# albertgassol1/vf-nerf

Hardware: AMD Instinct MI355X
Metric: rays/sec (4096-ray chunk, 128 samples/ray) + PSNR vs ref (higher is better)
Workload: dtype f16x3+f32acc

## Files before the change

### vf_nerf_amd/csrc/vfn_mlp16.hip

```cpp
#include <string.h>
#include <utility>
#include "vfn_common.h"
#include "vfn_plan.h"

typedef _Float16 half8 __attribute__((ext_vector_type(8)));
typedef _Float16 half2v __attribute__((ext_vector_type(2)));
typedef float float2v __attribute__((ext_vector_type(2)));
typedef float f32x16 __attribute__((ext_vector_type(16)));
typedef float f32x4v __attribute__((ext_vector_type(4)));

#ifndef VFN16_ASCALE
#define VFN16_ASCALE 1
#endif
#define VFN16_WSCALE 64.0f
#define VFN16_INV_WSCALE 0.015625f
#define VFN16_PACK_WSCALE (VFN16_ASCALE ? 1.0f : VFN16_WSCALE)
#define VFN16_XSCALE (VFN16_ASCALE ? VFN16_WSCALE : 1.0f)
#ifndef VFN16_SAVE_AUX
#define VFN16_SAVE_AUX 2
#endif
#ifndef VFN16_HANDOVER_NUM
#define VFN16_HANDOVER_NUM 8
#endif
#ifndef VFN16_DMA_STEPS
#define VFN16_DMA_STEPS 16
#endif
#ifndef VFN16_EPI_PER_MFMA
#define VFN16_EPI_PER_MFMA 6
#endif
#ifndef VFN16_EPI_PER_MFMA2
#define VFN16_EPI_PER_MFMA2 9
#endif
#ifndef VFN16_LATE_STORES
// ... 236 lines not shown
constexpr int rn_off_kb(int h) { int o = 0; for (int i = 0; i < h; ++i) o += RN_TILES[i] * chunk_kb(RN_ACT[i], RN_AUX[i]); return o; }

struct ChunkD { int net, off_kb, kb, aux; };
constexpr ChunkD chunk_of(int mode, int c) {
    if (!(mode & M16_BLKIN)) {
        const int vf_layers = (mode & M16_FEAT) ? 9 : 8;
        for (int h = 0; h < vf_layers; ++h) {
            if (c < VF_TILES[h]) return {0, vf_off_kb(h) + c * chunk_kb(VF_ACT[h], VF_AUX[h]), chunk_kb(VF_ACT[h], VF_AUX[h]), VF_AUX[h]};
            c -= VF_TILES[h];
        }
        if (c == 0) return {0, vf_off_kb(9), HEAD_KB, 0};
        c -= 1;
    }
    if (mode & M16_RENDER) {
        for (int h = 0; h < 4; ++h) {
            if (c < RN_TILES[h]) return {1, rn_off_kb(h) + c * chunk_kb(RN_ACT[h], RN_AUX[h]), chunk_kb(RN_ACT[h], RN_AUX[h]), RN_AUX[h]};
            c -= RN_TILES[h];
        }
        if (c == 0) return {1, rn_off_kb(4), HEAD_KB, 0};
    }
    return {0, 0, 0, 0};
}

constexpr int rn_first_chunk(int mode) { return (mode & M16_BLKIN) ? 0 : 72; }
constexpr bool chunk_two(int mode, int c) { return (mode & M16_C2) && !(mode & M16_BLKIN) && c >= 63 && c != 71; }
constexpr bool mode_one(int mode) { return (mode & M16_P1) != 0; }
#ifndef VFN16_P1_RING
#define VFN16_P1_RING 5
#endif
#define VFN16_P1_SLOT_KB 20
constexpr int ring_of(int mode) { return mode_one(mode) ? VFN16_P1_RING : 3; }
constexpr int slot_u4(int mode) { return mode_one(mode) ? VFN16_P1_SLOT_KB * 64 : VFN16_MAX_CHUNK_KB * 64; }
constexpr int slot_base(int mode, int c) { return (c % ring_of(mode)) * slot_u4(mode); }
static_assert(VFN16_P1_RING * VFN16_P1_SLOT_KB <= 3 * VFN16_MAX_CHUNK_KB, "the single-product ring must fit into the split modes' ring");
constexpr int stores_of(int mode, int c) { return (c == 0 || ((mode & M16_RENDER) && c == rn_first_chunk(mode))) ? 0 : 4; }
constexpr int young_ops(int mode, int c) {
    const int ring = ring_of(mode);
    int n = 0;
    for (int k = (c - ring + 2 > 0 ? c - ring + 2 : 0); k < c; ++k) n += stores_of(mode, k);
    for (int j = 2; j <= ring - 2; ++j)
        if (c + j >= ring - 1 && chunk_of(mode, c + j).kb > 0) n += (((chunk_of(mode, c + j).kb - 1) / 2 + 1) / VFN16_WAVES);
    return n;
}

struct Mlp16Args {
    const uint4* vf_w;
    const uint4* rn_w;
    const float* points;
    const float* ray_dirs;
    float* out_vec;
    float* out_colors;
    long long n_points;
    int dirs_div;
    int vf_multires, rn_multires;
    uint32_t vf_bytes, rn_bytes;
    float* saved;
    float* save_aux_vf;
    float* save_aux_rn;
    uint32_t* save_masks;
    int save_f16;
    uint4* blk_out;
    const uint4* blk_in;
    const float* vec_in;
    const int* src;
    const int* out_index;
    long long ws_first, ws_points;
// ... 164 lines not shown
        typedef unsigned int u32x16 __attribute__((ext_vector_type(16)));
        const u32x16 u = __builtin_bit_cast(u32x16, cy.pend);
        constexpr int N = 16 / PARTS;
        if constexpr (PART == 0) b = 0;
#pragma unroll
        for (int r = 15 - PART * N; r > 15 - (PART + 1) * N; --r) b = __builtin_amdgcn_alignbit(b, u[r] + 0x7fffffffu, 31);
        if constexpr (PART == PARTS - 1) cy.lm[TILE >> 1] |= b << (16 * (TILE & 1));
    }
}
template <int SLOT>
__device__ __forceinline__ void store_mask(const Pipe16& p, Carry16& cy) {
    typedef unsigned int u32x4 __attribute__((ext_vector_type(4)));
    const __amdgpu_buffer_rsrc_t rs = __builtin_amdgcn_make_buffer_rsrc(
        reinterpret_cast<unsigned char*>(p.masks) + (size_t)SLOT * p.mask_bytes, 0, (int)p.mask_bytes, 0x00020000);
    const u32x4 w = {cy.lm[0], cy.lm[1], cy.lm[2], cy.lm[3]};
    __builtin_amdgcn_raw_buffer_store_b128(w, rs, (int)p.mask_voff, 0, 0);
    cy.lm[0] = 0; cy.lm[1] = 0; cy.lm[2] = 0; cy.lm[3] = 0;
}

template <int TILE>
__device__ __forceinline__ void store_blocks(const Pipe16& p, const X16& x) {
    typedef unsigned int u32x4 __attribute__((ext_vector_type(4)));
    const __amdgpu_buffer_rsrc_t rs = __builtin_amdgcn_make_buffer_rsrc(p.blk_out, 0, (int)p.blk_bytes, 0x00020000);
#pragma unroll
    for (int s = 0; s < 2; ++s) {
        __builtin_amdgcn_raw_buffer_store_b128(__builtin_bit_cast(u32x4, x.hi[2 * TILE + s]), rs, (int)p.blk_voff, (2 * TILE + s) * 2048, 0);
        __builtin_amdgcn_raw_buffer_store_b128(__builtin_bit_cast(u32x4, x.lo[2 * TILE + s]), rs, (int)p.blk_voff, (2 * TILE + s) * 2048 + 1024, 0);
    }
}

template <int MODE, int C0, int ACT, int AUX, int NCH, int EPI, int PEPI, int PKB, int SLOT = -1, int PSLOT = -1, bool BLK = false,
          bool PBLK = false>
__device__ __forceinline__ void layer16(const X16& xin, const A16& aux, X16& xout, X16& xpend, Carry16& cy, float (&head)[3],
                                       const Pipe16& p, int wave, int lane) {
    constexpr int NKB = ACT + AUX;
    constexpr int E = NKB / 2 > 0 ? NKB / 2 : 1;
    constexpr int H = NKB * VFN16_HANDOVER_NUM / 16 > 0 ? NKB * VFN16_HANDOVER_NUM / 16 : 1;
    constexpr int PMAX = (VFN16_MAX_CHUNK_KB + VFN16_WAVES - 1) / VFN16_WAVES;
    constexpr int DSPAN = NKB - H > 0 ? NKB - H : 1;
    constexpr int DSTEPS = DSPAN < VFN16_DMA_STEPS ? DSPAN : VFN16_DMA_STEPS;
    static_assert(PEPI < 0 || PKB >= E, "the pending tile must be complete before it is read");
    constexpr bool TRAIN = (MODE & M16_TRAIN) != 0;
    constexpr bool LATE = TRAIN && VFN16_LATE_STORES;
    constexpr int DEND = LATE ? (NKB - 4 > H + 1 ? NKB - 4 : (H + 1 < NKB ? H + 1 : NKB - 1)) : 0;
    constexpr int SBEG = LATE ? DEND : H;
    constexpr int SSTEPS = LATE ? (NKB - DEND > 0 ? NKB - DEND : 1) : (DSPAN < 4 ? DSPAN : 4);
    constexpr int DST = LATE ? (DEND - H > 0 ? DEND - H : 1) : DSTEPS;
    constexpr int MPARTS = (LATE && E <= H) ? (DEND - H >= 4 ? 4 : (DEND - H >= 2 ? 2 : (DEND - H >= 1 ? 1 : 0))) : 0;
    static_for<NCH>([&](auto ich) {
        constexpr int ch = decltype(ich)::value;
        constexpr int C = C0 + ch;
        constexpr int RING = ring_of(MODE);
        constexpr ChunkD dcur = chunk_of(MODE, C), dnext = chunk_of(MODE, C + 1), ddma = chunk_of(MODE, C + RING - 1);
        static_assert(dcur.kb == 2 * NKB + 1, "layer shape and chunk table disagree");
        constexpr bool P1 = mode_one(MODE);
        constexpr bool W2 = chunk_two(MODE, C);
        constexpr bool D2 = chunk_two(MODE, C + RING - 1) || P1;
        constexpr int DNKB = (ddma.kb - 1) / 2;
        constexpr int DPIECES = P1 ? DNKB + 1 : (D2 ? DNKB + ddma.aux + 1 : ddma.kb);
        auto piece_blk = [&](int idx) -> int {
            if (P1) return idx < DNKB ? 2 * idx : 2 * DNKB;
            if (!D2) return idx;
            if (ddma.aux == 0) return 2 * idx;
            return idx < DNKB ? 2 * idx : (idx < DNKB + ddma.aux ? 2 * (idx - ddma.aux) + 1 : 2 * DNKB);
        };
        constexpr int PM = D2 ? (DPIECES + VFN16_WAVES - 1) / VFN16_WAVES : PMAX;
        const uint4* cb = p.lds + slot_base(MODE, C);
        constexpr int FB = P1 ? 1 : 2;
        f32x16 acc = cy.bias;
        half8 fh[VFN16_FDEPTH], fl[VFN16_FDEPTH];
        fh[0] = cy.fh0;
        if (!P1 && (!W2 || ACT == 0)) fl[0] = cy.fl0;
        if (VFN16_FDEPTH == 3 && NKB > 1) {
            fh[1] = __builtin_bit_cast(half8, cb[FB * 64 + lane]);
            if (!W2 && !P1) fl[1] = __builtin_bit_cast(half8, cb[3 * 64 + lane]);
        }
        half8 ehi[2], elo[2];
        [[maybe_unused]] unsigned mbits = 0;
#pragma unroll
        for (int st = 0; st < NKB; ++st) {
            constexpr int AHEAD = VFN16_FDEPTH - 1;
            if (st + AHEAD < NKB) {
                fh[(st + AHEAD) % VFN16_FDEPTH] = __builtin_bit_cast(half8, cb[(FB * (st + AHEAD)) * 64 + lane]);
                if (!P1 && (!W2 || st + AHEAD >= ACT)) fl[(st + AHEAD) % VFN16_FDEPTH] = __builtin_bit_cast(half8, cb[(2 * (st + AHEAD) + 1) * 64 + lane]);
            }
            const half8 a_hi = fh[st % VFN16_FDEPTH];
            const half8 x_hi = st < ACT ? xin.hi[st < ACT ? st : 0] : aux.hi[st >= ACT ? st - ACT : 0];
            const half8 x_lo = st < ACT ? xin.lo[st < ACT ? st : 0] : aux.lo[st >= ACT ? st - ACT : 0];
            acc = __builtin_amdgcn_mfma_f32_32x32x16_f16(a_hi, x_hi, acc, 0, 0, 0);
#ifndef ABL_P1
// ... 4 lines not shown
#endif
#ifdef ABL_NOEPI
            if (st == 0 && (ch > 0 || PEPI >= 0)) asm volatile("" :: "v"(cy.pend));
            if (false) {
#else
            if (st < E && (ch > 0 || PEPI >= 0)) {
#endif
#pragma unroll
                for (int pr = st * 8 / E; pr < (st + 1) * 8 / E; ++pr) {
                    const int sblk = pr >> 2, j = (pr & 3) * 2;
                    if (ch > 0) epi_pair<EPI, TRAIN, !P1>(cy.pend, cy.sat, pr, ehi[sblk], elo[sblk], j);
                    else epi_pair<(PEPI >= 0 ? PEPI : 0), TRAIN, !P1>(cy.pend, cy.sat, pr, ehi[sblk], elo[sblk], j);
                    if ((pr & 3) == 3) {
                        asm volatile("" : "+a"(ehi[sblk]));
                        if constexpr (!P1) asm volatile("" : "+a"(elo[sblk]));
                        if (ch > 0) { xout.hi[2 * (ch > 0 ? ch - 1 : 0) + sblk] = ehi[sblk]; if constexpr (!P1) xout.lo[2 * (ch > 0 ? ch - 1 : 0) + sblk] = elo[sblk]; }
                        else { xpend.hi[PKB + sblk] = ehi[sblk]; if constexpr (!P1) xpend.lo[PKB + sblk] = elo[sblk]; }
                    }
                }
#ifndef VFN16_NOGROUPS
                if constexpr (!P1) {
                __builtin_amdgcn_sched_group_barrier(0x100, W2 ? 1 : 2, 0);
                __builtin_amdgcn_sched_group_barrier(0x008, 1, 0);
                __builtin_amdgcn_sched_group_barrier(0x002, W2 ? VFN16_EPI_PER_MFMA2 : VFN16_EPI_PER_MFMA, 0);
                __builtin_amdgcn_sched_group_barrier(0x008, 1, 0);
                __builtin_amdgcn_sched_group_barrier(0x002, W2 ? VFN16_EPI_PER_MFMA2 : VFN16_EPI_PER_MFMA, 0);
                if (!W2) {
                    __builtin_amdgcn_sched_group_barrier(0x008, 1, 0);
                    __builtin_amdgcn_sched_group_barrier(0x002, VFN16_EPI_PER_MFMA, 0);
                }
                }
#endif
            }
            if (st == H - 1 && dnext.kb > 0) {
#ifndef ABL_NOSYNC
#ifdef ABL_LOOSE_WAIT
                if ((MODE & M16_TRAIN) != 0) asm volatile("s_waitcnt vmcnt(4)" ::: "memory");
                else
#endif
                if constexpr (P1 && LATE) {
                    constexpr int young = young_ops(MODE, C);
                    static_assert(young < 64, "vmcnt is a 6-bit field");
                    if constexpr (young == 0) asm volatile("s_waitcnt vmcnt(0)" ::: "memory");
                    else asm volatile("s_waitcnt vmcnt(%0)" :: "n"(young) : "memory");
                } else
                if (LATE && C > 0 && (ch == 0 || ch > 1 || PEPI >= 0)) asm volatile("s_waitcnt vmcnt(4)" ::: "memory");
                else asm volatile("s_waitcnt vmcnt(0)" ::: "memory");
                __builtin_amdgcn_s_barrier();
#endif
            }
#ifndef ABL_NODMA
            if (st >= H && st < H + DST && ddma.kb > 0) {
#pragma unroll
                for (int i = (st - H) * PM / DST; i < (st - H + 1) * PM / DST; ++i) {
                    if (VFN16_WAVES * i + VFN16_WAVES <= DPIECES) dma_piece<ddma.net, ddma.off_kb, slot_base(MODE, C + RING - 1)>(p, piece_blk(wave + VFN16_WAVES * i), lane, P1 ? wave + VFN16_WAVES * i : -1);
                    else if (VFN16_WAVES * i < DPIECES) {
                        const int idx = min(wave + VFN16_WAVES * i, DPIECES - 1);
                        dma_piece<ddma.net, ddma.off_kb, slot_base(MODE, C + RING - 1)>(p, piece_blk(idx), lane, P1 ? idx : -1);
                    }
                }
            }
#endif
#ifndef ABL_NOMASK
            if (TRAIN && MPARTS > 0 && st >= H && st < H + MPARTS && (ch > 0 || PEPI >= 0)) {
                static_for<MPARTS>([&](auto ip) {
                    constexpr int part = decltype(ip)::value;
                    if (st - H == part) {
                        if (ch > 0) collect_mask_part<(ch > 0 ? ch - 1 : 0), EPI, part, (MPARTS > 0 ? MPARTS : 1)>(cy, mbits);
                        else collect_mask_part<PKB / 2, (PEPI >= 0 ? PEPI : 0), part, (MPARTS > 0 ? MPARTS : 1)>(cy, mbits);
                    }
                });
            }
#endif
            if (TRAIN && st >= SBEG && st < SBEG + SSTEPS && (ch > 0 || PEPI >= 0)) {
#ifndef ABL_NOMASK
                if (st == (LATE ? SBEG : VFN16_MASK_STEP(H, NKB))) {
                    if constexpr (MPARTS > 0) {
                        if (ch == 0) store_mask<(PSLOT >= 0 ? PSLOT : 0)>(p, cy);
                    } else {
                        if (ch > 0) collect_mask<(ch > 0 ? ch - 1 : 0), EPI>(cy);
                        else { collect_mask<PKB / 2, (PEPI >= 0 ? PEPI : 0)>(cy); store_mask<(PSLOT >= 0 ? PSLOT : 0)>(p, cy); }
                    }
                }
#endif
#pragma unroll
                for (int q = (st - SBEG) * 4 / SSTEPS; q < (st - SBEG + 1) * 4 / SSTEPS; ++q) {
                    if (ch > 0) save_group<(SLOT >= 0 ? SLOT : 0), (ch > 0 ? ch - 1 : 0), (MODE & M16_SF16) != 0>(p, cy.pend, q);
                    else save_group<(PSLOT >= 0 ? PSLOT : 0), PKB / 2, (MODE & M16_SF16) != 0>(p, cy.pend, q);
                }
            }
            if (st == H && ((BLK && ch > 0) || (PBLK && ch == 0))) {
                if (ch > 0) store_blocks<(ch > 0 ? ch - 1 : 0)>(p, xout);
                else store_blocks<PKB / 2>(p, xpend);
            }
            if (st == NKB - 1 && dnext.kb > 0) prefetch_chunk<MODE, (dnext.kb > 0 ? C + 1 : C)>(cy, p, lane);
#ifndef VFN16_NOSCHED
            __builtin_amdgcn_sched_barrier(0);
#endif
        }
        if (EPI == EPI_RELU || EPI == EPI_TANH) {
            cy.pend = acc;
#if VFN16_RANGE_TRACK == 2
            if (EPI == EPI_RELU) {
                float mx = fmaxf(acc[0], acc[1]);
#pragma unroll
                for (int r = 2; r < 16; r += 2) mx = fmaxf(mx, fmaxf(acc[r], acc[r + 1]));
                cy.sat |= __builtin_amdgcn_ballot_w64(mx >= VFN16_CLAMP);
            }
#endif
        } else {
#pragma unroll
            for (int c = 0; c < 3; ++c) {
                const float v = acc[c] * VFN16_INV_WSCALE;
                head[c] = (EPI == EPI_HEAD_TANH) ? tanh_exp(v) : 1.0f / (1.0f + expf(-v));
            }
        }
    });
}

__device__ __forceinline__ float enc_value(const float (&x)[3], const float (&sn)[18], const float (&cs)[18], int multires, int k) {
    if (k < 3) return x[k];
    const int idx = k - 3, oct = idx / 6, rem = idx - 6 * oct;
    if (oct >= multires) return 0.f;
    return rem < 3 ? sn[3 * oct + rem] : cs[3 * oct + rem - 3];
}

template <typename F>
__device__ __forceinline__ void build_aux(A16& aux, int g, F col, float& ain) {
// ... 42 lines not shown
#pragma unroll
    for (int j = 0; j < 3; ++j)
#pragma unroll
        for (int c = 0; c < 3; ++c) {
            float s = 0.f, k = 0.f;
            if (2 * j < multires) {
                sincosf(x[c] * (g ? (float)(2 << (2 * j)) : (float)(1 << (2 * j))), &s, &k);
                if (2 * j + g >= multires) { s = 0.f; k = 0.f; }
            }
            const float so = __shfl_xor(s, 32, 64), ko = __shfl_xor(k, 32, 64);
            sn[6 * j + c] = g ? so : s;          cs[6 * j + c] = g ? ko : k;
            sn[6 * j + 3 + c] = g ? s : so;      cs[6 * j + 3 + c] = g ? k : ko;
        }
}

template <int MODE>
__device__ __forceinline__ void render_aux(const Mlp16Args& a, A16& aux, const float (&xr)[3], const float (&dr)[3], const float (&nrm)[3],
                                           long long m, bool in, int g, float& ain) {
    const int rn_multires = a.rn_multires;
    float sn[18], cs[18];
    encode_sincos(dr, rn_multires, g, sn, cs);
    const int ncol = 6 + 6 * rn_multires;
    auto rn_col = [&](int k) -> float {
        if (k < 3) return xr[k];
        if (k >= ncol) return k < ncol + 3 ? nrm[k - ncol] : 0.f;
        return enc_value(dr, sn, cs, rn_multires, k - 3);
    };
    build_aux(aux, g, rn_col, ain);
    if ((MODE & M16_TRAIN) && in) save_aux(a.save_aux_rn, m, g, rn_col);
}

template <int MODE>
__device__ __forceinline__ void render_tail(const Mlp16Args& a, const Pipe16& p, Carry16& cy, X16& xa, X16& xb, const A16& aux,
                                            const float (&nrm)[3], long long m, bool in, int wave, int lane) {
    constexpr int R = EPI_RELU, NONE = -1;
    constexpr int C0 = rn_first_chunk(MODE);
    float rgb[3] = {0.f, 0.f, 0.f};
    layer16<MODE, C0 + 0, 16, 3, 8, R, NONE, 0, 9, -1>(xb, aux, xa, xb, cy, rgb, p, wave, lane);
    layer16<MODE, C0 + 8, 16, 0, 8, R, R, 14, 10, 9>(xa, aux, xb, xa, cy, rgb, p, wave, lane);
    layer16<MODE, C0 + 16, 16, 0, 8, R, R, 14, 11, 10>(xb, aux, xa, xb, cy, rgb, p, wave, lane);
    layer16<MODE, C0 + 24, 16, 0, 8, R, R, 14, 12, 11>(xa, aux, xb, xa, cy, rgb, p, wave, lane);
    layer16<MODE, C0 + 32, 16, 0, 1, EPI_HEAD_SIGMOID, R, 14, -1, 12>(xb, aux, xa, xb, cy, rgb, p, wave, lane);
    const long long mo = m;
    if (in && (threadIdx.x & 32) == 0) {
        a.out_vec[mo * 3 + 0] = nrm[0]; a.out_vec[mo * 3 + 1] = nrm[1]; a.out_vec[mo * 3 + 2] = nrm[2];
        a.out_colors[mo * 3 + 0] = rgb[0]; a.out_colors[mo * 3 + 1] = rgb[1]; a.out_colors[mo * 3 + 2] = rgb[2];
    }
}

__device__ __forceinline__ void report_range(const Mlp16Args& a, unsigned long long sat, float ain) {
    if (a.status) {
        const unsigned bits = (sat != 0ull ? 1u : 0u) | (ain >= VFN16_CLAMP ? 2u : 0u);
        if (bits) atomicOr(a.status, bits);
    }
}

template <int MODE>
__global__ __launch_bounds__(256, 1) void vfn_mlp16_kernel(const Mlp16Args a) {
    __shared__ __attribute__((aligned(16))) uint4 s_ring[3 * VFN16_SLOT + 256 * 8];
    float* s_park = reinterpret_cast<float*>(s_ring + 3 * VFN16_SLOT) + threadIdx.x * 32;
    const int tid = threadIdx.x;
    const int lane = tid & 63;
    const int wave = __builtin_amdgcn_readfirstlane(tid >> 6);
    const int g = lane >> 5;
#ifdef VFN16_STAMPS
    const unsigned long long st_t0 = __builtin_amdgcn_s_memtime(), st_r0 = __builtin_amdgcn_s_memrealtime();
#endif
    unsigned long long ck_t0 = 0ull, ck_r0 = 0ull;
    if constexpr ((MODE & M16_RENDER) != 0 && (MODE & M16_BLKIN) == 0 && (MODE & M16_TRAIN) == 0) {
        if (a.clock) { ck_t0 = __builtin_amdgcn_s_memtime(); ck_r0 = __builtin_amdgcn_s_memrealtime(); }
    }
    const long long m = (long long)blockIdx.x * VFN16_PTS + wave * 32 + (lane & 31);
    long long n_live = a.n_points;
    if (a.n_dev) {
        const long long nd = (long long)*a.n_dev;
        n_live = nd < n_live ? nd : n_live;
        if ((long long)blockIdx.x * VFN16_PTS >= n_live) return;
    }
    const bool in = m < n_live;

    if constexpr ((MODE & M16_BLKIN) != 0) {
        const int dpos = in ? a.src[m] : -1;
        const bool live = dpos >= 0;
        float xr[3] = {0.f, 0.f, 0.f}, dr[3] = {0.f, 0.f, 0.f}, nrm[3] = {0.f, 0.f, 0.f};
        if (live) {
            const long long di = dpos / a.dirs_div;
#pragma unroll
            for (int c = 0; c < 3; ++c) { xr[c] = a.points[(long long)dpos * 3 + c]; dr[c] = a.ray_dirs[di * 3 + c]; nrm[c] = a.vec_in[m * 3 + c]; }
        }
        Pipe16 p;
        p.lds = s_ring;
        p.vf_w = __builtin_amdgcn_make_buffer_rsrc(const_cast<uint4*>(a.rn_w), 0, (int)a.rn_bytes, 0x00020000);
        p.rn_w = p.vf_w;
        p.saved = nullptr; p.slot_floats = 0; p.slot_bytes = 0; p.save_voff = 0; p.blk_out = nullptr; p.blk_bytes = 0; p.blk_voff = 0;
        p.masks = nullptr; p.mask_bytes = 0; p.mask_voff = 0; p.save16 = 0; p.save_voff16 = 0; p.feat_voff = 0; p.st_tile = 0; p.st_q = 0;
        dma_chunk<MODE, 0>(p, wave, lane);
        dma_chunk<MODE, 1>(p, wave, lane);
        X16 xa, xb;
        A16 aux;
        float ain_blk = 0.f;
        {
            typedef unsigned int u32x4 __attribute__((ext_vector_type(4)));
            const __amdgpu_buffer_rsrc_t rs_blk = __builtin_amdgcn_make_buffer_rsrc(
                const_cast<uint4*>(a.blk_in), 0, (int)(((a.n_points + 31) & ~31ll) * 1024), 0x00020000);
            const unsigned goff = in ? (unsigned)((m >> 5) * 32768 + lane * 16) : 0xfffffff0u;
            u32x4 q[32];
#pragma unroll
            for (int i = 0; i < 32; ++i) q[i] = __builtin_amdgcn_raw_buffer_load_b128(rs_blk, goff, i * 1024, 0);
            render_aux<MODE>(a, aux, xr, dr, nrm, -1, false, g, ain_blk);
#pragma unroll
            for (int t = 0; t < 8; ++t) {
                half8 h0 = __builtin_bit_cast(half8, q[4 * t + 0]), l0 = __builtin_bit_cast(half8, q[4 * t + 1]);
                half8 h1 = __builtin_bit_cast(half8, q[4 * t + 2]), l1 = __builtin_bit_cast(half8, q[4 * t + 3]);
                asm volatile("" : "+a"(h0)); asm volatile("" : "+a"(l0)); asm volatile("" : "+a"(h1)); asm volatile("" : "+a"(l1));
                xb.hi[2 * t] = h0; xb.lo[2 * t] = l0; xb.hi[2 * t + 1] = h1; xb.lo[2 * t + 1] = l1;
            }
        }
        asm volatile("s_waitcnt vmcnt(0)" ::: "memory");
        __builtin_amdgcn_s_barrier();
        Carry16 cy;
#pragma unroll
        for (int q = 0; q < 16; ++q) cy.pend[q] = 0.f;
        cy.lm[0] = 0; cy.lm[1] = 0; cy.lm[2] = 0; cy.lm[3] = 0; cy.sat = 0ull;
        prefetch_chunk<MODE, 0>(cy, p, lane);
#ifdef VFN16_STAMPS
        const unsigned long long st_t1 = __builtin_amdgcn_s_memtime();
#endif
        render_tail<MODE>(a, p, cy, xa, xb, aux, nrm, live ? (long long)dpos : -1, live, wave, lane);
        report_range(a, cy.sat, ain_blk);
#ifdef VFN16_STAMPS
        if (threadIdx.x == 0 && live) {
            const unsigned long long t2 = __builtin_amdgcn_s_memtime(), r2 = __builtin_amdgcn_s_memrealtime();
            a.out_colors[(long long)dpos * 3 + 0] = (float)(st_t1 - st_t0); a.out_colors[(long long)dpos * 3 + 1] = (float)(t2 - st_t0);
            a.out_colors[(long long)dpos * 3 + 2] = (float)(r2 - st_r0);
        }
#endif
    } else {
    float x[3] = {0.f, 0.f, 0.f};
    if (in) { x[0] = a.points[m * 3 + 0]; x[1] = a.points[m * 3 + 1]; x[2] = a.points[m * 3 + 2]; }
    float d[3] = {0.f, 0.f, 0.f};
    int out_row = -1;
    if ((MODE & M16_RENDER) && in) {
        const long long di = m / a.dirs_div;
        d[0] = a.ray_dirs[di * 3 + 0]; d[1] = a.ray_dirs[di * 3 + 1]; d[2] = a.ray_dirs[di * 3 + 2];
        if (a.out_index) out_row = a.out_index[m];
    }
    asm volatile("s_waitcnt vmcnt(0)" ::: "memory");
    if (MODE & M16_RENDER) {
        s_park[0] = x[0]; s_park[1] = x[1]; s_park[2] = x[2];
        s_park[4] = d[0]; s_park[5] = d[1]; s_park[6] = d[2];
    }

    Pipe16 p;
    p.lds = s_ring;
    p.vf_w = __builtin_amdgcn_make_buffer_rsrc(const_cast<uint4*>(a.vf_w), 0, (int)a.vf_bytes, 0x00020000);
    p.rn_w = __builtin_amdgcn_make_buffer_rsrc(const_cast<uint4*>((MODE & M16_RENDER) ? a.rn_w : a.vf_w), 0,
                                               (int)((MODE & M16_RENDER) ? a.rn_bytes : a.vf_bytes), 0x00020000);
    const bool frag = (a.save_f16 & 2) != 0;
    const long long mw = m + a.ws_first;
    p.slot_floats = frag ? ((a.ws_points + 31) >> 5) * 8192 : a.ws_points * 256;
    p.saved = a.saved + a.ws_first * 256;
    {
        const long long left = p.slot_floats * 4 - a.ws_first * 1024;
        p.slot_bytes = (uint32_t)(left < 0x7fffffffll ? left : 0x7fffffffll);
    }
    p.save_voff = !in ? (frag ? 0xc0000000u : 0xfffffff0u) : (frag ? (uint32_t)((m >> 5) * 32768 + lane * 16) : (uint32_t)(m * 1024 + g * 16));
    p.save_voff16 = !in ? (frag ? 0xc0000000u : 0xfffffff0u) : (frag ? (uint32_t)((m >> 5) * 32768 + lane * 8) : (uint32_t)(m * 1024 + g * 8));
    p.feat_voff = in ? (uint32_t)(m * 1024 + g * 16) : 0xfffffff0u;
    p.st_tile = frag ? 4096u : 128u; p.st_q = frag ? 1024u : 32u;
    p.masks = a.save_masks; p.mask_bytes = (uint32_t)(a.ws_points * 32); p.mask_voff = in ? (uint32_t)((2 * mw + g) * 16) : 0xfffffff0u;
    p.save16 = a.save_f16 & 1;
    p.blk_out = a.blk_out; p.blk_bytes = (uint32_t)(((a.n_points + 31) & ~31ll) * 1024);
    p.blk_voff = (uint32_t)((m >> 5) * 32768 + lane * 16);
    dma_chunk<MODE, 0>(p, wave, lane);
    dma_chunk<MODE, 1>(p, wave, lane);
    if constexpr (mode_one(MODE)) static_for<VFN16_P1_RING - 3>([&](auto ic) { dma_chunk<MODE, 2 + decltype(ic)::value>(p, wave, lane); });
#ifdef ABL_NODMA
    dma_chunk<MODE, 9>(p, wave, lane);
    dma_chunk<MODE, 10>(p, wave, lane);
    dma_chunk<MODE, 11>(p, wave, lane);
#endif

    const int vf_multires = a.vf_multires;
    A16 aux;
    float ain = 0.f;
    {
        float sn[18], cs[18];
        encode_sincos(x, vf_multires, g, sn, cs);
        build_aux(aux, g, [&](int k) { return enc_value(x, sn, cs, vf_multires, k); }, ain);
        if ((MODE & M16_TRAIN) && in) save_aux(a.save_aux_vf, mw, g, [&](int k) { return enc_value(x, sn, cs, vf_multires, k); });
        half8* pk = reinterpret_cast<half8*>(s_park + 8);
#pragma unroll
        for (int q = 0; q < 3; ++q) { pk[2 * q] = aux.hi[q]; pk[2 * q + 1] = aux.lo[q]; }
    }
    asm volatile("s_waitcnt vmcnt(0)" ::: "memory");
    __builtin_amdgcn_s_barrier();
    Carry16 cy;
#pragma unroll
    for (int q = 0; q < 16; ++q) cy.pend[q] = 0.f;
    cy.lm[0] = 0; cy.lm[1] = 0; cy.lm[2] = 0; cy.lm[3] = 0; cy.sat = 0ull;
    prefetch_chunk<MODE, 0>(cy, p, lane);

    X16 xa, xb;
    float vec[3] = {0.f, 0.f, 0.f};
#ifdef VFN16_STAMPS
    const unsigned long long st_t1 = __builtin_amdgcn_s_memtime();
#endif
    constexpr int R = EPI_RELU, T = EPI_TANH, NONE = -1;
    layer16<MODE, 0, 0, 3, 8, R, NONE, 0, 0, -1>(xa, aux, xb, xb, cy, vec, p, wave, lane);
    layer16<MODE, 8, 16, 0, 8, R, R, 14, 1, 0>(xb, aux, xa, xb, cy, vec, p, wave, lane);
    layer16<MODE, 16, 16, 0, 8, R, R, 14, 2, 1>(xa, aux, xb, xa, cy, vec, p, wave, lane);
    layer16<MODE, 24, 16, 0, 7, R, R, 14, 3, 2>(xb, aux, xa, xb, cy, vec, p, wave, lane);
    { A16 ax; load_aux(ax, s_park); layer16<MODE, 31, 14, 3, 8, R, R, 12, 4, 3>(xa, ax, xb, xa, cy, vec, p, wave, lane); }
    layer16<MODE, 39, 16, 0, 8, R, R, 14, 5, 4>(xb, aux, xa, xb, cy, vec, p, wave, lane);
    layer16<MODE, 47, 16, 0, 8, R, R, 14, 6, 5>(xa, aux, xb, xa, cy, vec, p, wave, lane);
    layer16<MODE, 55, 16, 0, 8, R, R, 14, 7, 6>(xb, aux, xa, xb, cy, vec, p, wave, lane);
    if constexpr (!(MODE & M16_FEAT)) {
        layer16<MODE, 63, 16, 0, 1, EPI_HEAD_TANH, R, 14, -1, 7>(xa, aux, xb, xa, cy, vec, p, wave, lane);
        if (in && g == 0) { a.out_vec[m * 3 + 0] = vec[0]; a.out_vec[m * 3 + 1] = vec[1]; a.out_vec[m * 3 + 2] = vec[2]; }
        report_range(a, cy.sat, ain);
    } else {
    constexpr bool BO = (MODE & M16_BLKOUT) != 0;
    layer16<MODE, 63, 16, 0, 8, T, R, 14, 8, 7, BO, false>(xa, aux, xb, xa, cy, vec, p, wave, lane);
    layer16<MODE, 71, 16, 0, 1, EPI_HEAD_TANH, T, 14, -1, 8, false, BO>(xa, aux, xb, xb, cy, vec, p, wave, lane);
    if constexpr (!(MODE & M16_RENDER)) {
        if (in && g == 0) { a.out_vec[m * 3 + 0] = vec[0]; a.out_vec[m * 3 + 1] = vec[1]; a.out_vec[m * 3 + 2] = vec[2]; }
        report_range(a, cy.sat, ain);
#ifdef VFN16_STAMPS
        if (threadIdx.x == 0) {
            const unsigned long long t2 = __builtin_amdgcn_s_memtime(), r2 = __builtin_amdgcn_s_memrealtime();
            a.out_vec[m * 3 + 0] = (float)(st_t1 - st_t0); a.out_vec[m * 3 + 1] = (float)(t2 - st_t0); a.out_vec[m * 3 + 2] = (float)(r2 - st_r0);
        }
#endif
    } else {
    float nrm[3];
#pragma unroll
    for (int c = 0; c < 3; ++c) nrm[c] = __shfl(vec[c], lane & 31, 64);
    const float xr[3] = {s_park[0], s_park[1], s_park[2]};
    const float dr[3] = {s_park[4], s_park[5], s_park[6]};
    A16 raux;
    render_aux<MODE>(a, raux, xr, dr, nrm, (MODE & M16_TRAIN) ? mw : m, in, g, ain);
    render_tail<MODE>(a, p, cy, xa, xb, raux, nrm, a.out_index ? (long long)out_row : m, a.out_index ? out_row >= 0 : in, wave, lane);
    report_range(a, cy.sat, ain);
    if constexpr ((MODE & M16_TRAIN) == 0) {
        if (a.clock && threadIdx.x == 0 && (long long)blockIdx.x < a.clock_slots) {
            const unsigned long long t1 = __builtin_amdgcn_s_memtime(), r1 = __builtin_amdgcn_s_memrealtime();
            a.clock[2 * blockIdx.x] = t1 - ck_t0; a.clock[2 * blockIdx.x + 1] = r1 - ck_r0;
        }
    }
    const long long mo = (long long)blockIdx.x * VFN16_PTS + (threadIdx.x >> 6) * 32 + (threadIdx.x & 31);
    (void)mo;
#ifdef VFN16_STAMPS
    if (threadIdx.x == 0) {
        const unsigned long long t1 = __builtin_amdgcn_s_memtime(), r1 = __builtin_amdgcn_s_memrealtime();
        a.out_colors[mo * 3 + 0] = (float)(t1 - st_t0); a.out_colors[mo * 3 + 1] = (float)(r1 - st_r0);
    }
#endif
    }
    }
    }
}

int check_vf16(const Plan16& vf, const char* what) {
    bool ok = vf.feat_layer == 1 && vf.n_hidden == 9 && (int)vf.head_off_kb == vf_off_kb(9);
    for (int h = 0; ok && h < 9; ++h)
        ok = vf.act16[h] == VF_ACT[h] && vf.aux16[h] == VF_AUX[h] && vf.n_tiles[h] == VF_TILES[h] && (int)vf.off_kb[h] == vf_off_kb(h);
    if (!ok) { vfn_set_error("%s: the f16x3 kernels are specialised for the shipped vector-field network shape", what); return VFN_ERR_UNSUPPORTED; }
    return VFN_OK;
}
int check_rn16(const Plan16& rn, const char* what) {
    bool ok = rn.n_hidden == 4 && (int)rn.head_off_kb == rn_off_kb(4);
    for (int h = 0; ok && h < 4; ++h)
        ok = rn.act16[h] == RN_ACT[h] && rn.aux16[h] == RN_AUX[h] && rn.n_tiles[h] == RN_TILES[h] && (int)rn.off_kb[h] == rn_off_kb(h);
    if (!ok) { vfn_set_error("%s: the f16x3 kernels are specialised for the shipped rendering network shape", what); return VFN_ERR_UNSUPPORTED; }
    return VFN_OK;
}

}

static int check_kind16(int net_kind, const Plan16& p, const char* what) {
    return net_kind == VFN_NET_VF ? check_vf16(p, what) : check_rn16(p, what);
}

static thread_local uint32_t* t_status_word = nullptr;

uint32_t* vfn_internal_f16x3_status() { return t_status_word; }

extern "C" int vfn_f16x3_set_status(uint32_t* status_word) {
    t_status_word = status_word;
    return VFN_OK;
}

static thread_local unsigned long long* t_clock_probe = nullptr;
static thread_local long long t_clock_slots = 0;

extern "C" int vfn_f16x3_set_clock_probe(uint64_t* stamps, int64_t slots) {
    VFN_REQUIRE(slots >= 0 && (stamps || slots == 0), "vfn_f16x3_set_clock_probe: %lld slots without a buffer", (long long)slots);
    t_clock_probe = reinterpret_cast<unsigned long long*>(stamps);
    t_clock_slots = stamps ? slots : 0;
    return VFN_OK;
}

VfnReportScope::VfnReportScope(uint32_t* status_word, uint64_t* clock_stamps, int64_t clock_slots)
    : old_status(t_status_word), old_clock(t_clock_probe), old_slots(t_clock_slots) {
    if (status_word) t_status_word = status_word;
    if (clock_stamps && clock_slots > 0) { t_clock_probe = reinterpret_cast<unsigned long long*>(clock_stamps); t_clock_slots = clock_slots; }
}
VfnReportScope::~VfnReportScope() { t_status_word = old_status; t_clock_probe = old_clock; t_clock_slots = old_slots; }

extern "C" int vfn_vf_mlp16_fwd(const vfn_net_geom* geom, const void* packed16, const float* points, int64_t n_points,
                                 float* out_vec, void* stream) {
    Mlp16Args a = {};
    VfnNetPlan p32; Plan16 vf;
    int rc = make_plan16(VFN_NET_VF, geom, &p32, &vf, "vfn_vf_mlp16_fwd");
    if (rc != VFN_OK) return rc;
    rc = check_vf16(vf, "vfn_vf_mlp16_fwd");
    if (rc != VFN_OK) return rc;
    if (n_points <= 0) return VFN_OK;
    VFN_REQUIRE(packed16 && points && out_vec, "vfn_vf_mlp16_fwd: NULL argument");
    a.vf_w = (const uint4*)packed16; a.points = points; a.out_vec = out_vec; a.n_points = n_points; a.dirs_div = 1;
    a.vf_multires = vf.multires; a.vf_bytes = vf.total_kb * 1024u;
    a.status = t_status_word;
    a.clock = t_clock_probe; a.clock_slots = t_clock_slots;
    const long long blocks = (n_points + VFN16_PTS - 1) / VFN16_PTS;
    hipLaunchKernelGGL(vfn_mlp16_kernel<M16_VF_VEC>, dim3((unsigned)blocks), dim3(256), 0, (hipStream_t)stream, a);
    return vfn_check_launch("vfn_vf_mlp16_fwd");
}

static int launch_fused16(const char* what, const vfn_net_geom* vf_geom, const void* vf_packed16, const vfn_net_geom* rn_geom,
                          const void* rn_packed16, const float* points, const float* ray_dirs, int64_t n_points,
                          int32_t samples_per_ray, const int32_t* out_index, bool scatter, int32_t colour_products, float* normals,
                          float* colors, void* stream, const int32_t* n_dev = nullptr) {
    Mlp16Args a = {};
    a.n_dev = n_dev;
    VfnNetPlan p32; Plan16 vf, rn;
    VFN_REQUIRE(vf_geom && rn_geom, "%s: NULL argument", what);
    int rc = make_plan16(VFN_NET_VF, vf_geom, &p32, &vf, what);
    if (rc != VFN_OK) return rc;
    rc = make_plan16(VFN_NET_RENDER, rn_geom, &p32, &rn, what);
    if (rc != VFN_OK) return rc;
    rc = check_vf16(vf, what);
    if (rc != VFN_OK) return rc;
    rc = check_rn16(rn, what);
    if (rc != VFN_OK) return rc;
    VFN_REQUIRE(vf_geom->feature_dims == VFN_HIDDEN && rn_geom->feature_dims == VFN_HIDDEN, "%s: both nets need feature_dims == %d", what, VFN_HIDDEN);
    VFN_REQUIRE(colour_products == 2 || colour_products == 3, "%s: colour_products must be 2 or 3 (got %d)", what, colour_products);
    if (n_points <= 0) return VFN_OK;
    VFN_REQUIRE(vf_packed16 && rn_packed16 && points && ray_dirs && normals && colors && (out_index || !scatter), "%s: NULL argument", what);
    VFN_REQUIRE(samples_per_ray > 0, "%s: samples_per_ray must be > 0", what);
    a.vf_w = (const uint4*)vf_packed16; a.rn_w = (const uint4*)rn_packed16; a.points = points; a.ray_dirs = ray_dirs;
    a.out_vec = normals; a.out_colors = colors; a.out_index = out_index; a.n_points = n_points; a.dirs_div = samples_per_ray;
    a.vf_multires = vf.multires; a.rn_multires = rn.multires; a.vf_bytes = vf.total_kb * 1024u; a.rn_bytes = rn.total_kb * 1024u;
    a.status = t_status_word;
    a.clock = t_clock_probe; a.clock_slots = t_clock_slots;
    const long long blocks = (n_points + VFN16_PTS - 1) / VFN16_PTS;
    if (colour_products == 2) hipLaunchKernelGGL(vfn_mlp16_kernel<M16_FUSED | M16_C2>, dim3((unsigned)blocks), dim3(256), 0, (hipStream_t)stream, a);
    else hipLaunchKernelGGL(vfn_mlp16_kernel<M16_FUSED>, dim3((unsigned)blocks), dim3(256), 0, (hipStream_t)stream, a);
    return vfn_check_launch(what);
}

extern "C" int vfn_vf_render_fused16_fwd(const vfn_net_geom* vf_geom, const void* vf_packed16, const vfn_net_geom* rn_geom,
                                          const void* rn_packed16, const float* points, const float* ray_dirs,
                                          int64_t n_points, int32_t samples_per_ray, float* normals, float* colors,
                                          void* stream) {
    return launch_fused16("vfn_vf_render_fused16_fwd", vf_geom, vf_packed16, rn_geom, rn_packed16, points, ray_dirs, n_points, samples_per_ray,
                          nullptr, false, 3, normals, colors, stream);
}

extern "C" int vfn_vf_render_fused16_scatter(const vfn_net_geom* vf_geom, const void* vf_packed16, const vfn_net_geom* rn_geom,
                                          const void* rn_packed16, const float* points, const float* ray_dirs,
                                          int64_t n_points, int32_t samples_per_ray, const int32_t* out_index, float* normals,
                                          float* colors, void* stream) {
    return launch_fused16("vfn_vf_render_fused16_scatter", vf_geom, vf_packed16, rn_geom, rn_packed16, points, ray_dirs, n_points,
                          samples_per_ray, out_index, true, 3, normals, colors, stream);
}

extern "C" int vfn_vf_render_fused16_products(const vfn_net_geom* vf_geom, const void* vf_packed16, const vfn_net_geom* rn_geom,
                                              const void* rn_packed16, const float* points, const float* ray_dirs, int64_t n_points,
                                              int32_t samples_per_ray, const int32_t* out_index, int32_t colour_products,
                                              float* normals, float* colors, void* stream) {
    return launch_fused16("vfn_vf_render_fused16_products", vf_geom, vf_packed16, rn_geom, rn_packed16, points, ray_dirs, n_points,
                          samples_per_ray, out_index, false, colour_products, normals, colors, stream);
}

int vfn_internal_fused16_products_dev(const vfn_net_geom* vf_geom, const void* vf_packed16, const vfn_net_geom* rn_geom, const void* rn_packed16,
                                      const float* points, const float* ray_dirs, int64_t n_points, const int32_t* n_dev, int32_t samples_per_ray,
                                      const int32_t* out_index, int32_t colour_products, float* normals, float* colors, void* stream) {
    return launch_fused16("vfn_render_fwd (colour branch on the selected samples)", vf_geom, vf_packed16, rn_geom, rn_packed16, points, ray_dirs,
// ... 147 lines not shown
```

Baseline: 2.056 million.

## Make fused MLP kernel persistent and carry weight ring across point groups

Launches one block per CU and loops each block over point groups instead of launching one block per group. For fused modes where the chunk count is a multiple of the LDS ring size, the weight DMA for the next group's first chunks is issued during the previous group's tail, so the weight pipeline never drains between groups. Saturation reporting is gathered once per block. This risks lower occupancy (one block per CU) and load imbalance in exchange for avoiding the per-block refill of the weight ring.

```diff
diff --git a/vf_nerf_amd/csrc/vfn_mlp16.hip b/vf_nerf_amd/csrc/vfn_mlp16.hip
--- a/vf_nerf_amd/csrc/vfn_mlp16.hip
+++ b/vf_nerf_amd/csrc/vfn_mlp16.hip
@@ -1,4 +1,5 @@
 #include <string.h>
+#include <atomic>
 #include <utility>
 #include "vfn_common.h"
 #include "vfn_plan.h"
@@ -301,6 +302,11 @@
 constexpr int ring_of(int mode) { return mode_one(mode) ? VFN16_P1_RING : 3; }
 constexpr int slot_u4(int mode) { return mode_one(mode) ? VFN16_P1_SLOT_KB * 64 : VFN16_MAX_CHUNK_KB * 64; }
 constexpr int slot_base(int mode, int c) { return (c % ring_of(mode)) * slot_u4(mode); }
+constexpr int n_chunks(int mode) { int c = 0; while (chunk_of(mode, c).kb > 0) ++c; return c; }
+constexpr bool mode_persistent(int mode) { return (mode & (M16_TRAIN | M16_BLKOUT | M16_BLKIN)) == 0; }
+constexpr bool ring_closes(int mode) { return mode_persistent(mode) && n_chunks(mode) % ring_of(mode) == 0; }
+static_assert(n_chunks(M16_FUSED) == 105 && ring_closes(M16_FUSED) && ring_closes(M16_FUSED | M16_C2) && !ring_closes(M16_VF_VEC),
+              "fused passes carry the ring across the group boundary, vector-only passes refill it");
 static_assert(VFN16_P1_RING * VFN16_P1_SLOT_KB <= 3 * VFN16_MAX_CHUNK_KB, "the single-product ring must fit into the split modes' ring");
 constexpr int stores_of(int mode, int c) { return (c == 0 || ((mode & M16_RENDER) && c == rn_first_chunk(mode))) ? 0 : 4; }
 constexpr int young_ops(int mode, int c) {
@@ -531,7 +537,7 @@
 template <int MODE, int C0, int ACT, int AUX, int NCH, int EPI, int PEPI, int PKB, int SLOT = -1, int PSLOT = -1, bool BLK = false,
           bool PBLK = false>
 __device__ __forceinline__ void layer16(const X16& xin, const A16& aux, X16& xout, X16& xpend, Carry16& cy, float (&head)[3],
-                                       const Pipe16& p, int wave, int lane) {
+                                       const Pipe16& p, int wave, int lane, bool more = false) {
     constexpr int NKB = ACT + AUX;
     constexpr int E = NKB / 2 > 0 ? NKB / 2 : 1;
     constexpr int H = NKB * VFN16_HANDOVER_NUM / 16 > 0 ? NKB * VFN16_HANDOVER_NUM / 16 : 1;
@@ -550,11 +556,15 @@
         constexpr int ch = decltype(ich)::value;
         constexpr int C = C0 + ch;
         constexpr int RING = ring_of(MODE);
-        constexpr ChunkD dcur = chunk_of(MODE, C), dnext = chunk_of(MODE, C + 1), ddma = chunk_of(MODE, C + RING - 1);
+        constexpr int NCHK = n_chunks(MODE);
+        constexpr bool NWRAP = ring_closes(MODE) && C + 1 >= NCHK, DWRAP = ring_closes(MODE) && C + RING - 1 >= NCHK;
+        constexpr int CN = NWRAP ? C + 1 - NCHK : C + 1, CD = DWRAP ? C + RING - 1 - NCHK : C + RING - 1;
+        static_assert(slot_base(MODE, CD) == slot_base(MODE, C + RING - 1) && slot_base(MODE, CN) == slot_base(MODE, C + 1), "ring rotation");
+        constexpr ChunkD dcur = chunk_of(MODE, C), dnext = chunk_of(MODE, CN), ddma = chunk_of(MODE, CD);
         static_assert(dcur.kb == 2 * NKB + 1, "layer shape and chunk table disagree");
         constexpr bool P1 = mode_one(MODE);
         constexpr bool W2 = chunk_two(MODE, C);
-        constexpr bool D2 = chunk_two(MODE, C + RING - 1) || P1;
+        constexpr bool D2 = chunk_two(MODE, CD) || P1;
         constexpr int DNKB = (ddma.kb - 1) / 2;
         constexpr int DPIECES = P1 ? DNKB + 1 : (D2 ? DNKB + ddma.aux + 1 : ddma.kb);
         auto piece_blk = [&](int idx) -> int {
@@ -625,7 +635,7 @@
                 }
 #endif
             }
-            if (st == H - 1 && dnext.kb > 0) {
+            if (st == H - 1 && dnext.kb > 0 && (!NWRAP || more)) {
 #ifndef ABL_NOSYNC
 #ifdef ABL_LOOSE_WAIT
                 if ((MODE & M16_TRAIN) != 0) asm volatile("s_waitcnt vmcnt(4)" ::: "memory");
@@ -643,13 +653,13 @@
 #endif
             }
 #ifndef ABL_NODMA
-            if (st >= H && st < H + DST && ddma.kb > 0) {
+            if (st >= H && st < H + DST && ddma.kb > 0 && (!DWRAP || more)) {
 #pragma unroll
                 for (int i = (st - H) * PM / DST; i < (st - H + 1) * PM / DST; ++i) {
-                    if (VFN16_WAVES * i + VFN16_WAVES <= DPIECES) dma_piece<ddma.net, ddma.off_kb, slot_base(MODE, C + RING - 1)>(p, piece_blk(wave + VFN16_WAVES * i), lane, P1 ? wave + VFN16_WAVES * i : -1);
+                    if (VFN16_WAVES * i + VFN16_WAVES <= DPIECES) dma_piece<ddma.net, ddma.off_kb, slot_base(MODE, CD)>(p, piece_blk(wave + VFN16_WAVES * i), lane, P1 ? wave + VFN16_WAVES * i : -1);
                     else if (VFN16_WAVES * i < DPIECES) {
                         const int idx = min(wave + VFN16_WAVES * i, DPIECES - 1);
-                        dma_piece<ddma.net, ddma.off_kb, slot_base(MODE, C + RING - 1)>(p, piece_blk(idx), lane, P1 ? idx : -1);
+                        dma_piece<ddma.net, ddma.off_kb, slot_base(MODE, CD)>(p, piece_blk(idx), lane, P1 ? idx : -1);
                     }
                 }
             }
@@ -686,7 +696,7 @@
                 if (ch > 0) store_blocks<(ch > 0 ? ch - 1 : 0)>(p, xout);
                 else store_blocks<PKB / 2>(p, xpend);
             }
-            if (st == NKB - 1 && dnext.kb > 0) prefetch_chunk<MODE, (dnext.kb > 0 ? C + 1 : C)>(cy, p, lane);
+            if (st == NKB - 1 && dnext.kb > 0 && !NWRAP) prefetch_chunk<MODE, (dnext.kb > 0 && !NWRAP ? C + 1 : C)>(cy, p, lane);
 #ifndef VFN16_NOSCHED
             __builtin_amdgcn_sched_barrier(0);
 #endif
@@ -795,15 +805,15 @@
 
 template <int MODE>
 __device__ __forceinline__ void render_tail(const Mlp16Args& a, const Pipe16& p, Carry16& cy, X16& xa, X16& xb, const A16& aux,
-                                            const float (&nrm)[3], long long m, bool in, int wave, int lane) {
+                                            const float (&nrm)[3], long long m, bool in, int wave, int lane, bool more = false) {
     constexpr int R = EPI_RELU, NONE = -1;
     constexpr int C0 = rn_first_chunk(MODE);
     float rgb[3] = {0.f, 0.f, 0.f};
     layer16<MODE, C0 + 0, 16, 3, 8, R, NONE, 0, 9, -1>(xb, aux, xa, xb, cy, rgb, p, wave, lane);
     layer16<MODE, C0 + 8, 16, 0, 8, R, R, 14, 10, 9>(xa, aux, xb, xa, cy, rgb, p, wave, lane);
     layer16<MODE, C0 + 16, 16, 0, 8, R, R, 14, 11, 10>(xb, aux, xa, xb, cy, rgb, p, wave, lane);
-    layer16<MODE, C0 + 24, 16, 0, 8, R, R, 14, 12, 11>(xa, aux, xb, xa, cy, rgb, p, wave, lane);
-    layer16<MODE, C0 + 32, 16, 0, 1, EPI_HEAD_SIGMOID, R, 14, -1, 12>(xb, aux, xa, xb, cy, rgb, p, wave, lane);
+    layer16<MODE, C0 + 24, 16, 0, 8, R, R, 14, 12, 11>(xa, aux, xb, xa, cy, rgb, p, wave, lane, more);
+    layer16<MODE, C0 + 32, 16, 0, 1, EPI_HEAD_SIGMOID, R, 14, -1, 12>(xb, aux, xa, xb, cy, rgb, p, wave, lane, more);
     const long long mo = m;
     if (in && (threadIdx.x & 32) == 0) {
         a.out_vec[mo * 3 + 0] = nrm[0]; a.out_vec[mo * 3 + 1] = nrm[1]; a.out_vec[mo * 3 + 2] = nrm[2];
@@ -827,7 +837,7 @@
     const int wave = __builtin_amdgcn_readfirstlane(tid >> 6);
     const int g = lane >> 5;
 #ifdef VFN16_STAMPS
-    const unsigned long long st_t0 = __builtin_amdgcn_s_memtime(), st_r0 = __builtin_amdgcn_s_memrealtime();
+    [[maybe_unused]] unsigned long long st_t0 = __builtin_amdgcn_s_memtime(), st_r0 = __builtin_amdgcn_s_memrealtime();
 #endif
     unsigned long long ck_t0 = 0ull, ck_r0 = 0ull;
     if constexpr ((MODE & M16_RENDER) != 0 && (MODE & M16_BLKIN) == 0 && (MODE & M16_TRAIN) == 0) {
@@ -841,6 +851,10 @@
         if ((long long)blockIdx.x * VFN16_PTS >= n_live) return;
     }
     const bool in = m < n_live;
+    constexpr bool PERSIST = mode_persistent(MODE);
+    constexpr bool CLOSED = ring_closes(MODE);
+    const long long n_groups = (n_live + VFN16_PTS - 1) / VFN16_PTS;
+    const long long g_step = PERSIST ? (long long)gridDim.x : n_groups;
 
     if constexpr ((MODE & M16_BLKIN) != 0) {
         const int dpos = in ? a.src[m] : -1;
@@ -899,6 +913,19 @@
         }
 #endif
     } else {
+    Pipe16 p;
+    p.lds = s_ring;
+    p.vf_w = __builtin_amdgcn_make_buffer_rsrc(const_cast<uint4*>(a.vf_w), 0, (int)a.vf_bytes, 0x00020000);
+    p.rn_w = __builtin_amdgcn_make_buffer_rsrc(const_cast<uint4*>((MODE & M16_RENDER) ? a.rn_w : a.vf_w), 0,
+                                               (int)((MODE & M16_RENDER) ? a.rn_bytes : a.vf_bytes), 0x00020000);
+    if constexpr (CLOSED) { dma_chunk<MODE, 0>(p, wave, lane); dma_chunk<MODE, 1>(p, wave, lane); }
+    unsigned long long sat_all = 0ull;
+    float ain = 0.f;
+    long long grp = blockIdx.x;
+    do {
+    const bool more = CLOSED && grp + g_step < n_groups;
+    const long long m = grp * VFN16_PTS + wave * 32 + (lane & 31);
+    const bool in = m < n_live;
     float x[3] = {0.f, 0.f, 0.f};
     if (in) { x[0] = a.points[m * 3 + 0]; x[1] = a.points[m * 3 + 1]; x[2] = a.points[m * 3 + 2]; }
     float d[3] = {0.f, 0.f, 0.f};
@@ -914,11 +941,6 @@
         s_park[4] = d[0]; s_park[5] = d[1]; s_park[6] = d[2];
     }
 
-    Pipe16 p;
-    p.lds = s_ring;
-    p.vf_w = __builtin_amdgcn_make_buffer_rsrc(const_cast<uint4*>(a.vf_w), 0, (int)a.vf_bytes, 0x00020000);
-    p.rn_w = __builtin_amdgcn_make_buffer_rsrc(const_cast<uint4*>((MODE & M16_RENDER) ? a.rn_w : a.vf_w), 0,
-                                               (int)((MODE & M16_RENDER) ? a.rn_bytes : a.vf_bytes), 0x00020000);
     const bool frag = (a.save_f16 & 2) != 0;
     const long long mw = m + a.ws_first;
     p.slot_floats = frag ? ((a.ws_points + 31) >> 5) * 8192 : a.ws_points * 256;
@@ -935,8 +957,11 @@
     p.save16 = a.save_f16 & 1;
     p.blk_out = a.blk_out; p.blk_bytes = (uint32_t)(((a.n_points + 31) & ~31ll) * 1024);
     p.blk_voff = (uint32_t)((m >> 5) * 32768 + lane * 16);
-    dma_chunk<MODE, 0>(p, wave, lane);
-    dma_chunk<MODE, 1>(p, wave, lane);
+    if constexpr (!CLOSED) {
+        if constexpr (PERSIST) __builtin_amdgcn_s_barrier();
+        dma_chunk<MODE, 0>(p, wave, lane);
+        dma_chunk<MODE, 1>(p, wave, lane);
+    }
     if constexpr (mode_one(MODE)) static_for<VFN16_P1_RING - 3>([&](auto ic) { dma_chunk<MODE, 2 + decltype(ic)::value>(p, wave, lane); });
 #ifdef ABL_NODMA
     dma_chunk<MODE, 9>(p, wave, lane);
@@ -946,7 +971,6 @@
 
     const int vf_multires = a.vf_multires;
     A16 aux;
-    float ain = 0.f;
     {
         float sn[18], cs[18];
         encode_sincos(x, vf_multires, g, sn, cs);
@@ -981,14 +1005,14 @@
     if constexpr (!(MODE & M16_FEAT)) {
         layer16<MODE, 63, 16, 0, 1, EPI_HEAD_TANH, R, 14, -1, 7>(xa, aux, xb, xa, cy, vec, p, wave, lane);
         if (in && g == 0) { a.out_vec[m * 3 + 0] = vec[0]; a.out_vec[m * 3 + 1] = vec[1]; a.out_vec[m * 3 + 2] = vec[2]; }
-        report_range(a, cy.sat, ain);
+        sat_all |= cy.sat;
     } else {
     constexpr bool BO = (MODE & M16_BLKOUT) != 0;
     layer16<MODE, 63, 16, 0, 8, T, R, 14, 8, 7, BO, false>(xa, aux, xb, xa, cy, vec, p, wave, lane);
     layer16<MODE, 71, 16, 0, 1, EPI_HEAD_TANH, T, 14, -1, 8, false, BO>(xa, aux, xb, xb, cy, vec, p, wave, lane);
     if constexpr (!(MODE & M16_RENDER)) {
         if (in && g == 0) { a.out_vec[m * 3 + 0] = vec[0]; a.out_vec[m * 3 + 1] = vec[1]; a.out_vec[m * 3 + 2] = vec[2]; }
-        report_range(a, cy.sat, ain);
+        sat_all |= cy.sat;
 #ifdef VFN16_STAMPS
         if (threadIdx.x == 0) {
             const unsigned long long t2 = __builtin_amdgcn_s_memtime(), r2 = __builtin_amdgcn_s_memrealtime();
@@ -1003,24 +1027,27 @@
     const float dr[3] = {s_park[4], s_park[5], s_park[6]};
     A16 raux;
     render_aux<MODE>(a, raux, xr, dr, nrm, (MODE & M16_TRAIN) ? mw : m, in, g, ain);
-    render_tail<MODE>(a, p, cy, xa, xb, raux, nrm, a.out_index ? (long long)out_row : m, a.out_index ? out_row >= 0 : in, wave, lane);
-    report_range(a, cy.sat, ain);
+    render_tail<MODE>(a, p, cy, xa, xb, raux, nrm, a.out_index ? (long long)out_row : m, a.out_index ? out_row >= 0 : in, wave, lane, more);
+    sat_all |= cy.sat;
     if constexpr ((MODE & M16_TRAIN) == 0) {
-        if (a.clock && threadIdx.x == 0 && (long long)blockIdx.x < a.clock_slots) {
+        if (a.clock) {
             const unsigned long long t1 = __builtin_amdgcn_s_memtime(), r1 = __builtin_amdgcn_s_memrealtime();
-            a.clock[2 * blockIdx.x] = t1 - ck_t0; a.clock[2 * blockIdx.x + 1] = r1 - ck_r0;
-        }
-    }
-    const long long mo = (long long)blockIdx.x * VFN16_PTS + (threadIdx.x >> 6) * 32 + (threadIdx.x & 31);
-    (void)mo;
+            if (threadIdx.x == 0 && grp < a.clock_slots) { a.clock[2 * grp] = t1 - ck_t0; a.clock[2 * grp + 1] = r1 - ck_r0; }
+            ck_t0 = t1; ck_r0 = r1;
+        }
+    }
 #ifdef VFN16_STAMPS
-    if (threadIdx.x == 0) {
+    {
         const unsigned long long t1 = __builtin_amdgcn_s_memtime(), r1 = __builtin_amdgcn_s_memrealtime();
-        a.out_colors[mo * 3 + 0] = (float)(t1 - st_t0); a.out_colors[mo * 3 + 1] = (float)(r1 - st_r0);
-    }
-#endif
-    }
-    }
+        if (threadIdx.x == 0) { a.out_colors[grp * VFN16_PTS * 3 + 0] = (float)(t1 - st_t0); a.out_colors[grp * VFN16_PTS * 3 + 1] = (float)(r1 - st_r0); }
+        st_t0 = t1; st_r0 = r1;
+    }
+#endif
+    }
+    }
+    grp += g_step;
+    } while (PERSIST && grp < n_groups);
+    report_range(a, sat_all, ain);
     }
 }
 
@@ -1071,6 +1098,19 @@
 }
 VfnReportScope::~VfnReportScope() { t_status_word = old_status; t_clock_probe = old_clock; t_clock_slots = old_slots; }
 
+static long long persistent_grid(long long groups) {
+    enum { MAX_DEV = 64 };
+    static std::atomic<int> s_cus[MAX_DEV];
+    int dev = 0;
+    if (hipGetDevice(&dev) != hipSuccess || dev < 0 || dev >= MAX_DEV) return groups;
+    int cus = s_cus[dev].load(std::memory_order_relaxed);
+    if (cus <= 0) {
+        if (hipDeviceGetAttribute(&cus, hipDeviceAttributeMultiprocessorCount, dev) != hipSuccess || cus <= 0) return groups;
+        s_cus[dev].store(cus, std::memory_order_relaxed);
+    }
+    return groups < cus ? groups : (long long)cus;
+}
+
 extern "C" int vfn_vf_mlp16_fwd(const vfn_net_geom* geom, const void* packed16, const float* points, int64_t n_points,
                                  float* out_vec, void* stream) {
     Mlp16Args a = {};
@@ -1085,7 +1125,7 @@
     a.vf_multires = vf.multires; a.vf_bytes = vf.total_kb * 1024u;
     a.status = t_status_word;
     a.clock = t_clock_probe; a.clock_slots = t_clock_slots;
-    const long long blocks = (n_points + VFN16_PTS - 1) / VFN16_PTS;
+    const long long blocks = persistent_grid((n_points + VFN16_PTS - 1) / VFN16_PTS);
     hipLaunchKernelGGL(vfn_mlp16_kernel<M16_VF_VEC>, dim3((unsigned)blocks), dim3(256), 0, (hipStream_t)stream, a);
     return vfn_check_launch("vfn_vf_mlp16_fwd");
 }
@@ -1116,7 +1156,7 @@
     a.vf_multires = vf.multires; a.rn_multires = rn.multires; a.vf_bytes = vf.total_kb * 1024u; a.rn_bytes = rn.total_kb * 1024u;
     a.status = t_status_word;
     a.clock = t_clock_probe; a.clock_slots = t_clock_slots;
-    const long long blocks = (n_points + VFN16_PTS - 1) / VFN16_PTS;
+    const long long blocks = persistent_grid((n_points + VFN16_PTS - 1) / VFN16_PTS);
     if (colour_products == 2) hipLaunchKernelGGL(vfn_mlp16_kernel<M16_FUSED | M16_C2>, dim3((unsigned)blocks), dim3(256), 0, (hipStream_t)stream, a);
     else hipLaunchKernelGGL(vfn_mlp16_kernel<M16_FUSED>, dim3((unsigned)blocks), dim3(256), 0, (hipStream_t)stream, a);
     return vfn_check_launch(what);
```

Result: no change. 2.042 million (-0.6%).
